# Adamtaranto/mimeo

Hardware: AMD Instinct MI355X
Metric: Gbp-aligned/sec (mimeo self, 1 Gbp genome, --minIdt 80 --minLen 100 --minCov 3) (higher is better)
Workload: dtype int32

## Files before the change

mimeo_amd/csrc/k6.h:

```cpp
#pragma once
#include <algorithm>
#include <cstdio>
#include <cstdlib>
#include <vector>

#include "device_util.h"

namespace mimeo {

constexpr int32_t NEG = -(1 << 30);
constexpr int32_t NEGH = -(1 << 29);

struct Cell {
    int32_t s;
    uint32_t nm, nx;
};
struct HalfResult {
    int32_t score;
    uint32_t i, j, nm, nx, overflow;
    uint32_t maxcols, rows;
    uint32_t base_lo, base_hi;
};
struct DpJob {
    uint32_t group, at, aq;
// ... 108 lines not shown
            const uint32_t side = t >= (long long)an.x ? 1u : 0u;
            const uint2 ix = B.P.pidx[2u * (b0 + rank) + side];
            const bool traced = ix.x != PATH_UNTRACED;
            const uint32_t n = traced ? ix.y : 0u;
            const PathBlock *blk = B.P.blk + (traced ? ix.x : 0u);
            const uint32_t lo = blocks_upto(blk, n, t);
            PathBlock b{0, 0, 0};
            if (lo) b = blk[lo - 1];
            if (lo && t - (long long)b.t < (long long)b.len) {
                const long long d = (long long)b.q - (long long)b.t, k = dir > 0 ? d - d0 : d0 - d;
                if (k <= 0) kmin = max(kmin, k);
                if (k >= 0) kmax = min(kmax, k);
                c = dir > 0 ? (long long)b.t + b.len : (long long)b.t - 1;
            } else if (dir > 0) {
                c = lo < n ? (long long)blk[lo].t : (side == 0 ? (long long)an.x : (long long)o.tend);
            } else {
                c = lo ? (long long)b.t + b.len - 1 : (side == 1 ? (long long)an.x - 1 : (long long)o.tstart - 1);
            }
        } else if (dir > 0) {
            c = (long long)o.tstart > t ? (long long)o.tstart : K_INF;
        } else {
            c = (long long)o.tend <= t ? (long long)o.tend - 1 : -1;
        }
        nt = dir > 0 ? min(nt, c) : max(nt, c);
    }
    for (int o = 32; o > 0; o >>= 1) {
        kmin = max(kmin, __shfl_xor(kmin, o));
        kmax = min(kmax, __shfl_xor(kmax, o));
        const long long on = __shfl_xor(nt, o);
        nt = dir > 0 ? min(nt, on) : max(nt, on);
    }
    RowBound r;
    r.kmin = wave_uniform_ll(kmin); r.kmax = wave_uniform_ll(kmax);
    nt = wave_uniform_ll(nt);
    const long long nrow = dir > 0 ? nt - (long long)at + 1 : (long long)at - nt;
    r.next = nrow > 0xFFFFFFFEll ? 0xFFFFFFFFu : (uint32_t)nrow;
    r.any = (r.kmin > -K_INF || r.kmax < K_INF) ? 1u : 0u;
    return r;
}
__device__ __forceinline__ bool bounds_none(const BoundCtx &B, uint64_t b0, uint32_t nacc, uint32_t at, int dir) {
    bool hit = false;
    for (uint32_t e = threadIdx.x & 63u; e < nacc; e += 64u) {
        const mimeo_alignment o = B.aln[b0 + e];
        if (o.tend > o.tstart && (dir > 0 ? o.tend > at : o.tstart < at)) hit = true;
    }
    return __ballot(hit) == 0;
}

struct K6Buffers {
    DeviceBuf anchors, packed, jobs, res, cnt, astate, ovf_list, any;
    DeviceBuf pidx, accrank, arena, pool, tjobs, tres, tctr;
    DeviceBuf kjobs, pcnt, pslot, ptmp;
    DeviceBuf sweep;
};
extern K6Buffers g_k6;
int dp_round(Group *d_groups, uint32_t n, const mimeo_params *p, int32_t cap, bool bounded, const BoundCtx &bc, unsigned int *novf, unsigned int *nrestart);
int arena_reserve(uint64_t blocks, uint64_t used);
struct TraceStats { uint64_t arena_used, largest; float ms; uint32_t slices; };
int trace_round(Group *d_groups, const DpJob *d_jobs, uint32_t h0, const mimeo_params *p, int32_t cap, uint64_t budget, TraceStats &ts, bool bounded, BoundCtx bc);
int paths_pass(Group *d_groups, uint32_t ngroups, const mimeo_params *p, int32_t cap, const mimeo_alignment *d_aln, uint64_t budget, bool k6_stats);

}
```

mimeo_amd/csrc/k6_dp.hip:

```cpp
#include "k6_band.h"

namespace mimeo {

template <int WSTRIP>
__device__ __forceinline__ void load_qbits(const GStrandView &Q, uint32_t aq, int dir, uint32_t jb, uint32_t lenB,
                                           uint32_t &qlo, uint32_t &qhi, uint32_t &qn) {
    constexpr uint32_t SMASK = WSTRIP == 32 ? 0xFFFFFFFFu : ((1u << (WSTRIP & 31)) - 1u);
    if (jb > lenB) { qlo = qhi = qn = 0; return; }
    if (dir > 0) {
        int32_t p = (int32_t)(aq + jb) - 1;
        const Win32 w = win32(Q, p);
        qlo = w.lo & SMASK; qhi = w.hi & SMASK; qn = w.nm & SMASK;
    } else {
        int32_t p = (int32_t)aq - (int32_t)jb - (WSTRIP - 1);
        const Win32 w = win32(Q, p);
        qlo = __brev(w.lo & SMASK) >> (32 - WSTRIP); qhi = __brev(w.hi & SMASK) >> (32 - WSTRIP);
        qn = __brev(w.nm & SMASK) >> (32 - WSTRIP);
    }
}

struct RowBases { uint32_t lo, hi, nm; };
__device__ __forceinline__ RowBases load_row_bases(const GStrandView &T, uint32_t at, int dir, uint32_t i0) {
    if (dir > 0) {
        const Win32 w = win32(T, (int32_t)(at + i0 - 1u));
// ... 505 lines not shown
    return AnyRow{(int32_t *)b, (int32_t *)(b + ANY_COLS), b + 2u * ANY_COLS, b + 3u * ANY_COLS, b + 4u * ANY_COLS, b + 5u * ANY_COLS};
}
constexpr size_t ANY_SLOT_WORDS = 2u * 6u * (size_t)ANY_COLS;

struct CountRows {
    static constexpr uint32_t M = ANY_COLS - 1u, W = ANY_COLS;
    uint32_t *base;
    AnyRow P, N;
    __device__ __forceinline__ BandRows rows(uint32_t par, uint32_t, uint32_t) {
        P = any_row(base, par); N = any_row(base, par ^ 1u);
        return BandRows{P.cs, P.ds, N.cs, N.ds};
    }
    __device__ __forceinline__ void init(uint32_t j, int32_t c) {
        const AnyRow r0 = any_row(base, 0);
        r0.cs[j & M] = c; r0.cm[j & M] = 0; r0.cx[j & M] = 0;
        r0.ds[j & M] = NEG; r0.dm[j & M] = 0; r0.dx[j & M] = 0;
    }
    __device__ __forceinline__ Cell h(uint32_t j, bool dlive, bool dopen, bool diag, bool m, bool hd) const {
        Cell dd{0, 0, 0}, g{0, 0, 0};
        if (dlive) { dd.nm = P.dm[j & M]; dd.nx = P.dx[j & M]; }
        if (dopen) { dd.nm = P.cm[j & M]; dd.nx = P.cx[j & M]; }
        if (diag) { g.nm = P.cm[(j - 1) & M] + (m ? 1u : 0u); g.nx = P.cx[(j - 1) & M] + (m ? 0u : 1u); }
        N.dm[j & M] = dd.nm; N.dx[j & M] = dd.nx;
        const Cell hh = hd ? dd : g;
        N.cm[j & M] = hh.nm; N.cx[j & M] = hh.nx;
        return hh;
    }
    __device__ __forceinline__ Cell htag(uint32_t j) const { return Cell{0, N.cm[j & M], N.cx[j & M]}; }
    __device__ __forceinline__ Cell c(uint32_t j, const Cell &ht, const Cell &ia, bool ci) const { const Cell ct = ci ? ia : ht; N.cm[j & M] = ct.nm; N.cx[j & M] = ct.nx; return ct; }
};

template <bool BOUND>
__global__ __launch_bounds__(ANY_THREADS) void k6_dp_any(const Group *__restrict__ groups, const DpJob *__restrict__ jobs,
                                                         const unsigned int *__restrict__ list, uint32_t first,
                                                         HalfResult *__restrict__ res, uint32_t *__restrict__ scratch,
                                                         int32_t O, int32_t E, int32_t Y, int32_t cap, BoundCtx B,
                                                         HalfSweep *__restrict__ sweep) {
    const DpJob job = jobs[list[first + blockIdx.x]];
    const Group &G = groups[job.group];
    const uint32_t lenA = job.dir > 0 ? G.T.len - job.at : job.at;
    CountRows rows{scratch + (size_t)blockIdx.x * ANY_SLOT_WORDS};
    HalfSweep sw;
    const HalfResult r = band_dp<ANY_THREADS, BOUND>(rows, G, job, lenA, O, E, Y, cap, B, sw);
    if (threadIdx.x == 0) res[job.slot] = r;
    if (BOUND && threadIdx.x == 0) sweep[job.slot] = sw;
}

__global__ void k6_list_all(uint32_t n, unsigned int *__restrict__ novf, unsigned int *__restrict__ ovf_list) {
    const uint32_t k = blockIdx.x * blockDim.x + threadIdx.x;
    if (k < n) ovf_list[k] = k;
    if (k == 0) *novf = n;
}

int dp_round(Group *d_groups, uint32_t n, const mimeo_params *p, int32_t cap, bool bounded, const BoundCtx &bc,
                    unsigned int *novf, unsigned int *nrestart) {
    hipStream_t st = stream();
    int rc;
    const Group *groups = d_groups;
    const DpJob *jobs = (const DpJob *)g_k6.jobs.p;
    HalfResult *res = (HalfResult *)g_k6.res.p;
    HalfSweep *sweep = bounded ? (HalfSweep *)g_k6.sweep.p : nullptr;
    unsigned int *list = (unsigned int *)g_k6.ovf_list.p;
    const int32_t O = p->gap_open, E = p->gap_extend, Y = p->ydrop;
    const bool lean_ok = E <= (1 << 16) && O <= (1 << 24) && Y <= (1 << 28);
    if (bounded) {
        if (lean_ok) hipLaunchKernelGGL(k6_dp1_bounded, dim3(n), dim3(64), 0, st, groups, jobs, res, sweep, O, E, Y, bc, novf, list);
        else hipLaunchKernelGGL(k6_list_all, dim3((n + 255) / 256), dim3(256), 0, st, n, novf, list);
    } else {
        if (lean_ok) hipLaunchKernelGGL(k6_dp1, dim3(n), dim3(64), 0, st, groups, jobs, res, O, E, Y, nrestart);
        hipLaunchKernelGGL(k6_dp_wide, dim3(n), dim3(64), 0, st, groups, jobs, res, O, E, Y, novf, list, cap, lean_ok ? 0 : 1);
    }
    unsigned int nov = 0;
    HIP_TRY(hipMemcpyAsync(&nov, novf, 4, hipMemcpyDeviceToHost, st));
    HIP_TRY(hipStreamSynchronize(st));
    if (!nov) return 0;
    const unsigned int slots = std::min<unsigned int>(nov, 32u);
    if ((rc = g_k6.any.reserve((size_t)slots * ANY_SLOT_WORDS * 4))) return rc;
    const auto any = bounded ? k6_dp_any<true> : k6_dp_any<false>;
    for (unsigned int f = 0; f < nov; f += slots)
        hipLaunchKernelGGL(any, dim3(std::min(slots, nov - f)), dim3(ANY_THREADS), 0, st, groups, jobs, (const unsigned int *)list, f, res,
                           (uint32_t *)g_k6.any.p, O, E, Y, cap, bc, sweep);
    return 0;
}

}
```

mimeo_amd/csrc/k6_gapped.hip:

```cpp
#include "k6.h"

namespace mimeo {

constexpr uint32_t ANCHOR_W = 31, ANCHOR_CHUNK = 4096;
constexpr int ANCHOR_THREADS = 1024;

__device__ void wave_anchor_chunk(const GStrandView &T, const GStrandView &Q, const mimeo_hsp &h, uint32_t chunk,
                                  unsigned long long *packed) {
    const uint32_t lane = threadIdx.x & 63u, nw = h.length - ANCHOR_W + 1;
    const int32_t d = (int32_t)h.tstart - (int32_t)h.qstart;
    const uint32_t w0 = chunk * ANCHOR_CHUNK + lane * (ANCHOR_CHUNK / 64u), w1 = min(nw, w0 + ANCHOR_CHUNK / 64u);
    int32_t bs = INT32_MIN;
    uint32_t bw = 0xFFFFFFFFu;
    if (w0 < w1) {
        int32_t sum = 0;
        bool m;
        for (uint32_t k = 0; k < ANCHOR_W; k++) {
            int32_t pt = (int32_t)(h.tstart + w0 + k);
            sum += pair_score(T, Q, pt, pt - d, &m);
        }
        bs = sum; bw = w0;
        for (uint32_t w = w0 + 1; w < w1; w++) {
            int32_t add = (int32_t)(h.tstart + w + ANCHOR_W - 1), sub = (int32_t)(h.tstart + w - 1);
            sum += pair_score(T, Q, add, add - d, &m) - pair_score(T, Q, sub, sub - d, &m);
            if (sum > bs) { bs = sum; bw = w; }
        }
    }
    for (int o = 32; o > 0; o >>= 1) {
        int32_t ob = __shfl_xor(bs, o);
        uint32_t ow = __shfl_xor(bw, o);
        if (ob > bs || (ob == bs && ow < bw)) { bs = ob; bw = ow; }
    }
    if (lane == 0 && bw != 0xFFFFFFFFu)
        atomicMax(packed, ((unsigned long long)(uint32_t)(bs + 8192) << 32) | (unsigned long long)(0xFFFFFFFFu - bw));
}

constexpr uint32_t ANCHOR_SPLIT = 16;
__global__ __launch_bounds__(ANCHOR_THREADS) void k6_anchor_points(const Group *__restrict__ groups,
                                                                   const mimeo_hsp *__restrict__ hs,
                                                                   const uint32_t *__restrict__ order,
                                                                   unsigned long long *__restrict__ packed) {
    const Group &G = groups[blockIdx.x];
    const uint64_t b0 = G.hsp_begin;
    const uint32_t nw = gridDim.y * (ANCHOR_THREADS / 64), me = blockIdx.y * (ANCHOR_THREADS / 64) + (threadIdx.x >> 6);
    uint32_t item = 0;
    for (uint32_t r = 0; r < G.nchain; r++) {
        const mimeo_hsp h = hs[b0 + order[b0 + r]];
        if (h.length <= ANCHOR_W) continue;
        const uint32_t nch = (h.length - ANCHOR_W + 1 + ANCHOR_CHUNK - 1) / ANCHOR_CHUNK;
        const uint32_t first = (me + nw - item % nw) % nw;
        for (uint32_t c = first; c < nch; c += nw) wave_anchor_chunk(G.T, G.Q, h, c, &packed[b0 + r]);
        item += nch;
    }
}
__global__ __launch_bounds__(256) void k6_anchor_final(const Group *__restrict__ groups, const mimeo_hsp *__restrict__ hs,
                                                       const uint32_t *__restrict__ order,
                                                       const unsigned long long *__restrict__ packed,
                                                       uint2 *__restrict__ anchors) {
    const Group &G = groups[blockIdx.x];
    const uint64_t b0 = G.hsp_begin;
    for (uint32_t r = threadIdx.x; r < G.nchain; r += blockDim.x) {
        const mimeo_hsp h = hs[b0 + order[b0 + r]];
        uint32_t off = h.length / 2;
        if (h.length > ANCHOR_W) off = (0xFFFFFFFFu - (uint32_t)packed[b0 + r]) + ANCHOR_W / 2;
        anchors[b0 + r] = make_uint2(h.tstart + off, h.qstart + off);
    }
}

__device__ __forceinline__ bool in_boxes(const mimeo_alignment *aln, uint32_t n, uint2 a) {
    bool inside = false;
    for (uint32_t e = threadIdx.x & 63u; e < n; e += 64u) {
        const mimeo_alignment &o = aln[e];
        if (a.x >= o.tstart && a.x < o.tend && a.y >= o.qstart && a.y < o.qend) inside = true;
    }
    return __ballot(inside) != 0;
}

__device__ __forceinline__ bool on_half_path(const PathBlock *blk, uint32_t n, uint2 a) {
    const uint32_t lo = blocks_upto(blk, n, a.x);
    if (!lo) return false;
    const PathBlock b = blk[lo - 1];
    return a.x - b.t < b.len && a.y >= b.q && a.y - b.q == a.x - b.t;
}
__device__ __forceinline__ bool on_path(const PathView &P, const uint2 *anchors, uint64_t b0, uint32_t rank, uint2 a) {
    const uint2 an = anchors[b0 + rank];
    const uint2 ix = P.pidx[2u * (b0 + rank) + (a.x >= an.x ? 1u : 0u)];
    if (ix.x == PATH_UNTRACED) return false;
    return on_half_path(P.blk + ix.x, ix.y, a);
}
template <bool PATH>
__device__ __forceinline__ bool skip_test(const mimeo_alignment *aln, uint32_t n, uint2 a, const PathView &P,
                                          const uint2 *anchors, uint64_t b0) {
    if (!PATH) return in_boxes(aln + b0, n, a);
    bool on = false;
    for (uint32_t e = threadIdx.x & 63u; e < n; e += 64u) {
        const mimeo_alignment &o = aln[b0 + e];
        if (a.x >= o.tstart && a.x < o.tend && a.y >= o.qstart && a.y < o.qend && on_path(P, anchors, b0, P.accrank[b0 + e], a))
            on = true;
    }
    return __ballot(on) != 0;
}

enum : uint8_t { A_NEW = 0, A_DONE = 1, A_SKIPPED = 2, A_ACCEPTED = 3 };
constexpr uint32_t PICK_SCAN = 2048;
constexpr uint32_t NEAR_DIAG = 256, NEAR_POS = 8192, MAX_DEFER = 2;
constexpr uint32_t GUARD_FREE = 32, GUARD_DIAG = 4096, GUARD_COUNT = 4;

__device__ __forceinline__ uint32_t anchor_relation(uint2 a, uint2 b) {
    int32_t da = (int32_t)a.x - (int32_t)a.y, db = (int32_t)b.x - (int32_t)b.y;
    uint32_t dd = (uint32_t)abs(da - db), dp = a.x > b.x ? a.x - b.x : b.x - a.x;
    return ((dd <= NEAR_DIAG && dp <= NEAR_POS) ? 1u : 0u) | (dd <= GUARD_DIAG ? 2u : 0u);
}

template <bool PATH>
__global__ __launch_bounds__(64) void k6_pick(Group *__restrict__ groups, const uint2 *__restrict__ anchors,
                                              const mimeo_alignment *__restrict__ aln, uint32_t bmax,
                                              uint8_t *__restrict__ astate, uint8_t *__restrict__ adefer,
                                              DpJob *__restrict__ jobs, unsigned int *__restrict__ njobs, PathView P) {
    __shared__ uint32_t sb[MAX_BATCH];
    Group &G = groups[blockIdx.x];
    const uint64_t b0 = G.hsp_begin;
    const uint32_t first = G.next, lane = threadIdx.x;
    uint32_t nb = 0;
    for (uint32_t r = first; r < G.nchain && nb < bmax && r - first < PICK_SCAN; r++) {
        if (astate[b0 + r] != A_NEW) continue;
        const uint2 a = anchors[b0 + r];
        if (skip_test<PATH>(aln, G.nacc, a, P, anchors, b0)) {
            if (lane == 0) astate[b0 + r] = A_SKIPPED;
            continue;
        }
        uint32_t near = 0, band = 0;
        for (uint32_t r2 = first + lane; r2 < r; r2 += 64)
            if (astate[b0 + r2] == A_DONE) { const uint32_t x = anchor_relation(a, anchors[b0 + r2]); near |= x & 1u; band += x >> 1; }
        for (uint32_t k = lane; k < nb; k += 64) { const uint32_t x = anchor_relation(a, anchors[b0 + sb[k]]); near |= x & 1u; band += x >> 1; }
        if (__ballot(near) && adefer[b0 + r] < MAX_DEFER) {
            if (lane == 0) adefer[b0 + r]++;
            continue;
        }
        if (nb >= GUARD_FREE) {
            for (int o = 32; o > 0; o >>= 1) band += __shfl_xor(band, o);
            if (band >= GUARD_COUNT) continue;
        }
        if (lane == 0) sb[nb] = r;
        nb++;
        __syncthreads();
    }
    if (lane == 0) {
        G.nbatch = nb;
        unsigned int j0 = nb ? atomicAdd(njobs, 2u * nb) : 0u;
        G.job0 = j0;
        for (uint32_t k = 0; k < nb; k++) {
            const uint32_t r = sb[k];
            astate[b0 + r] = A_DONE;
            const uint2 a = anchors[b0 + r];
            const uint32_t slot = 2u * (uint32_t)(b0 + r);
            jobs[j0 + 2 * k] = DpJob{blockIdx.x, a.x, a.y, -1, slot, 0};
            jobs[j0 + 2 * k + 1] = DpJob{blockIdx.x, a.x, a.y, +1, slot + 1, 0};
        }
    }
}

constexpr uint32_t RESOLVE_NEW = 256;
static_assert(RESOLVE_NEW >= (uint32_t)MAX_BATCH, "k6_resolve accepts a full take in one invocation");

__device__ __forceinline__ bool bounds_touch(const PathView &P, const uint2 *anchors, uint64_t b0, uint32_t rank, uint4 o, uint2 a,
                                             const HalfResult &L, const HalfResult &R, const HalfSweep &sL, const HalfSweep &sR) {
    const uint32_t rowsL = L.rows ? L.rows : L.i, rowsR = R.rows ? R.rows : R.i;
    const long long tlo = (long long)a.x - rowsL, thi = (long long)a.x + rowsR;
    if ((long long)o.y <= tlo || (long long)o.x >= thi) return false;
    const long long d0 = (long long)a.y - (long long)a.x;
    bool hit = false;
    for (uint32_t side = 0; side < 2; side++) {
        const uint2 ix = P.pidx[2u * (b0 + rank) + side];
        if (ix.x == PATH_UNTRACED) continue;
        for (uint32_t k = threadIdx.x & 63u; k < ix.y; k += 64u) {
            const PathBlock b = P.blk[ix.x + k];
            const long long t0 = b.t, t1 = (long long)b.t + b.len, d = (long long)b.q - (long long)b.t;
            if (t0 < thi && t1 > (long long)a.x && d - d0 >= sR.klo && d - d0 <= sR.khi) hit = true;
            if (t0 < (long long)a.x && t1 > tlo && d0 - d >= sL.klo && d0 - d <= sL.khi) hit = true;
        }
    }
    return __ballot(hit) != 0;
}

template <bool PATH, bool BOUND = false, bool RANK = false>
__global__ __launch_bounds__(64) void k6_resolve(Group *__restrict__ groups, const uint2 *__restrict__ anchors,
                                                 const HalfResult *__restrict__ res, mimeo_alignment *__restrict__ aln,
                                                 uint8_t *__restrict__ astate, unsigned int *__restrict__ remaining, PathView P,
                                                 const HalfSweep *__restrict__ sweep) {
    __shared__ uint4 sbox[RESOLVE_NEW];
    __shared__ uint32_t srank[PATH ? RESOLVE_NEW : 1];
    Group &G = groups[blockIdx.x];
    const uint64_t b0 = G.hsp_begin;
    const uint32_t nacc0 = G.nacc;
    uint32_t nnew = 0, overflow = 0, r = G.next;
    for (; r < G.nchain; r++) {
        const uint8_t st = astate[b0 + r];
        if (st == A_SKIPPED || st == A_ACCEPTED) continue;
        if (nnew == RESOLVE_NEW) break;
        const uint2 a = anchors[b0 + r];
        bool inside = skip_test<PATH>(aln, nacc0, a, P, anchors, b0);
        if (!inside) {
            bool in2 = false;
            for (uint32_t e = threadIdx.x; e < nnew; e += 64) {
                uint4 o = sbox[e];
                if (a.x >= o.x && a.x < o.y && a.y >= o.z && a.y < o.w && (!PATH || on_path(P, anchors, b0, srank[PATH ? e : 0], a)))
                    in2 = true;
            }
            inside = __ballot(in2) != 0;
        }
// ... 103 lines not shown
            const uint32_t v = threadIdx.x >= o ? part[threadIdx.x - o] : 0u;
            __syncthreads();
            part[threadIdx.x] += v;
            __syncthreads();
        }
        if (g < ngroups) groups[g].job0 = carry + part[threadIdx.x] - n;
        __syncthreads();
        if (threadIdx.x == 1023) carry += part[1023];
        __syncthreads();
    }
}
__global__ __launch_bounds__(64) void k6_dense_copy(const Group *__restrict__ groups, const mimeo_alignment *__restrict__ aln,
                                                    mimeo_alignment *__restrict__ dense) {
    const Group &G = groups[blockIdx.x];
    for (uint32_t k = threadIdx.x; k < G.naln; k += 64) dense[G.job0 + k] = aln[G.hsp_begin + k];
}
void dense_alignments_device(Group *d_groups, uint32_t ngroups, const mimeo_alignment *d_aln, mimeo_alignment *d_dense) {
    hipLaunchKernelGGL(k6_dense_offsets, dim3(1), dim3(1024), 0, stream(), d_groups, ngroups);
    hipLaunchKernelGGL(k6_dense_copy, dim3(ngroups), dim3(64), 0, stream(), (const Group *)d_groups, d_aln, d_dense);
}

__global__ void k6_kept_ranks(Group *__restrict__ groups, uint32_t ngroups, const mimeo_alignment *__restrict__ aln,
                              uint32_t *__restrict__ accrank, const uint2 *__restrict__ pidx, int32_t thresh) {
    const uint32_t g = blockIdx.x * blockDim.x + threadIdx.x;
    if (g >= ngroups) return;
    Group &G = groups[g];
    const uint64_t b0 = G.hsp_begin;
    uint32_t k = 0;
    for (uint32_t e = 0; e < G.nacc; e++) {
        if (aln[b0 + e].score < thresh) continue;
        const uint32_t rank = accrank[b0 + e];
        const uint32_t slot = 2u * (uint32_t)(b0 + rank);
        if (pidx[slot].x == PATH_UNTRACED || pidx[slot + 1].x == PATH_UNTRACED) G.overflow = 1;
        accrank[b0 + k++] = rank;
    }
}

__global__ __launch_bounds__(256) void k6_ungapped_paths(const Group *__restrict__ groups, const mimeo_alignment *__restrict__ aln,
                                                         PathBlock *__restrict__ arena, uint2 *__restrict__ pidx,
                                                         uint32_t *__restrict__ accrank) {
    const Group &G = groups[blockIdx.x];
    const uint64_t b0 = G.hsp_begin;
    for (uint32_t r = threadIdx.x; r < G.nacc; r += 256) {
        const mimeo_alignment a = aln[b0 + r];
        arena[b0 + r] = PathBlock{a.tstart, a.qstart, a.tend - a.tstart};
        pidx[2u * (b0 + r)] = make_uint2((uint32_t)(b0 + r), 1u);
        pidx[2u * (b0 + r) + 1u] = make_uint2(0u, 0u);
        accrank[b0 + r] = r;
    }
}

K6Buffers g_k6;

static int round_stats(uint32_t n, uint64_t nhsps, bool bounded, unsigned long long *bound_jobs, const unsigned int *nrestart) {
    std::vector<DpJob> hj(n);
    std::vector<HalfResult> hall((size_t)nhsps * 2), hr(n);
    HIP_TRY(hipStreamSynchronize(stream()));
    HIP_TRY(hipMemcpy(hj.data(), g_k6.jobs.p, (size_t)n * sizeof(DpJob), hipMemcpyDeviceToHost));
    HIP_TRY(hipMemcpy(hall.data(), g_k6.res.p, hall.size() * sizeof(HalfResult), hipMemcpyDeviceToHost));
    for (size_t k = 0; k < hr.size(); k++) hr[k] = hall[hj[k].slot];
    unsigned long long hist[9] = {0}, rows = 0, maxr = 0, shortcut = 0;
    for (auto &r : hr) {
        if (!r.rows) { shortcut++; continue; }
        hist[std::min<uint32_t>(8, r.maxcols / 128)]++; rows += r.rows; maxr = std::max<unsigned long long>(maxr, r.rows);
    }
    unsigned long long rebased = 0;
    for (auto &r : hr) if (r.base_lo | r.base_hi) rebased++;
    unsigned int wide[2] = {0, 0};
    HIP_TRY(hipMemcpy(wide, nrestart, 8, hipMemcpyDeviceToHost));
    fprintf(stderr, "[k6] full strip width: restarted %u widened %u of %u\n", wide[0], wide[1], n);
    fprintf(stderr, "[k6] jobs %u shortcut %llu (rebased in k6_dp_any: %llu) rows total %llu max %llu band<128..>=1024:", n, shortcut, rebased, rows, maxr);
    for (int b = 0; b < 9; b++) fprintf(stderr, " %llu", hist[b]);
    fprintf(stderr, "\n");
    {
        unsigned long long fine[34] = {0};
        for (auto &r : hr) if (r.rows) fine[std::min<uint32_t>(33, r.maxcols / 32)]++;
        fprintf(stderr, "[k6] widest band, buckets of 32 columns from 448:");
        for (int b = 14; b < 34; b++) fprintf(stderr, " %llu", fine[b]);
        fprintf(stderr, "\n");
    }
    if (n <= 8)
        for (size_t k = 0; k < hr.size(); k++)
            fprintf(stderr, "  [k6] job %zu: dir %d rows %u maxcols %u i %u j %u rebased %d\n", k, hj[k].dir, hr[k].rows, hr[k].maxcols, hr[k].i, hr[k].j,
                    (hr[k].base_lo | hr[k].base_hi) ? 1 : 0);
    int shown = 0;
    for (auto &r : hr)
        if (!r.rows && shown < 8) { fprintf(stderr, "  [k6] zero-row job: score %d i %u j %u nm %u nx %u ovf %u\n", r.score, r.i, r.j, r.nm, r.nx, r.overflow); shown++; }
    if (bounded) {
        std::vector<HalfSweep> hs((size_t)nhsps * 2);
        HIP_TRY(hipMemcpy(hs.data(), g_k6.sweep.p, hs.size() * sizeof(HalfSweep), hipMemcpyDeviceToHost));
        for (auto &j : hj) *bound_jobs += hs[j.slot].nbound ? 1u : 0u;
    }
    return 0;
}

static int accepted_stats(const Group *d_groups, uint32_t ngroups, uint32_t bmax) {
    std::vector<Group> hg(ngroups);
    HIP_TRY(hipStreamSynchronize(stream()));
    HIP_TRY(hipMemcpy(hg.data(), d_groups, (size_t)ngroups * sizeof(Group), hipMemcpyDeviceToHost));
    unsigned long long hist[11] = {0}, sum = 0, over = 0;
    uint32_t mx = 0;
    for (const Group &g : hg) {
        uint32_t b = 0;
        while (b < 10 && (b ? 1u << (b - 1) : 0u) < g.nacc) b++;
        hist[b]++; sum += g.nacc; mx = std::max(mx, g.nacc); over += g.nacc > bmax ? 1u : 0u;
    }
    fprintf(stderr, "[k6] accepted per group: max %u mean %.2f of %u groups, %llu above the take of %u; 0 1 2 <=4 <=8 .. <=256 more:", mx,
            (double)sum / ngroups, ngroups, over, bmax);
    for (int b = 0; b < 11; b++) fprintf(stderr, " %llu", hist[b]);
    fprintf(stderr, "\n");
    return 0;
}

struct K6Call {
    uint32_t bmax, rounds;
    bool stats, path, bounded, box_paths;
    int32_t cap;
    uint64_t pool_budget;
    unsigned long long bound_jobs, rescheduled;
    TraceStats ts;
};

static int gapped_setup(Group *d_groups, uint32_t ngroups, const mimeo_hsp *d_sorted, const uint32_t *d_order, uint64_t nhsps, K6Call &c) {
    c.bmax = getenv("MIMEO_K6_BMAX") ? (uint32_t)atoi(getenv("MIMEO_K6_BMAX")) : K6_ROUND_ANCHORS / ngroups;
    c.bmax = c.bmax < 1 ? 1 : (c.bmax > MAX_BATCH ? MAX_BATCH : c.bmax);
    c.stats = getenv("MIMEO_K6_STATS") != nullptr;
    if (c.stats) fprintf(stderr, "[k6] take %u anchors per group and round (%u groups, limit %d, budget %u)\n", c.bmax, ngroups, MAX_BATCH, K6_ROUND_ANCHORS);
    c.cap = getenv("MIMEO_K6_SCORE_CAP") ? std::max(100000, atoi(getenv("MIMEO_K6_SCORE_CAP"))) : 2000000000;
    hipStream_t st = stream();
    int rc;
    if ((rc = g_k6.anchors.reserve(nhsps * sizeof(uint2)))) return rc;
    if ((rc = g_k6.packed.reserve(nhsps * 8))) return rc;
    HIP_TRY(hipMemsetAsync(g_k6.packed.p, 0, nhsps * 8, st));
    if ((rc = g_k6.jobs.reserve((size_t)ngroups * c.bmax * 2 * sizeof(DpJob)))) return rc;
    if ((rc = g_k6.res.reserve((size_t)nhsps * 2 * sizeof(HalfResult)))) return rc;
    if ((rc = g_k6.astate.reserve((size_t)nhsps * 2))) return rc;
    HIP_TRY(hipMemsetAsync(g_k6.astate.p, 0, (size_t)nhsps * 2, st));
    if ((rc = g_k6.cnt.reserve(32))) return rc;
    if ((rc = g_k6.ovf_list.reserve((size_t)ngroups * c.bmax * 2 * sizeof(unsigned int)))) return rc;
    const uint32_t asplit = ngroups > 4096 ? 1u : ANCHOR_SPLIT;
    hipLaunchKernelGGL(k6_anchor_points, dim3(ngroups, asplit), dim3(ANCHOR_THREADS), 0, st, (const Group *)d_groups,
                       d_sorted, d_order, (unsigned long long *)g_k6.packed.p);
    hipLaunchKernelGGL(k6_anchor_final, dim3(ngroups), dim3(256), 0, st, (const Group *)d_groups, d_sorted, d_order,
                       (const unsigned long long *)g_k6.packed.p, (uint2 *)g_k6.anchors.p);
    if (c.path || c.box_paths) {
        if ((rc = g_k6.tctr.reserve(16))) return rc;
        if ((rc = arena_reserve(1024, 0))) return rc;
        HIP_TRY(hipMemsetAsync(g_k6.tctr.p, 0, 16, st));
        size_t free_b = 0, total_b = 0;
        HIP_TRY(hipMemGetInfo(&free_b, &total_b));
        c.pool_budget = std::min<uint64_t>(((uint64_t)free_b + g_k6.pool.cap) / 4, 16ull << 30);
        if (getenv("MIMEO_K6_TRACE_POOL_MB")) c.pool_budget = (uint64_t)atol(getenv("MIMEO_K6_TRACE_POOL_MB")) << 20;
    }
    if (c.bounded && (rc = g_k6.sweep.reserve((size_t)nhsps * 2 * sizeof(HalfSweep)))) return rc;
    return 0;
}

static int gapped_rounds(Group *d_groups, uint32_t ngroups, uint64_t nhsps, const mimeo_params *p, mimeo_alignment *d_aln, K6Call &c) {
    hipStream_t st = stream();
    int rc;
    PathView pv{nullptr, nullptr, nullptr};
    if (c.path || c.box_paths) pv = PathView{(const uint2 *)g_k6.pidx.p, nullptr, (uint32_t *)g_k6.accrank.p};
    const auto pick = c.path ? k6_pick<true> : k6_pick<false>;
    const auto resolve = c.bounded ? k6_resolve<true, true> : c.path ? k6_resolve<true, false>
                         : c.box_paths ? k6_resolve<false, false, true> : k6_resolve<false, false>;
    const HalfSweep *sweep = c.bounded ? (const HalfSweep *)g_k6.sweep.p : nullptr;
    for (;;) {
        HIP_TRY(hipMemsetAsync(g_k6.cnt.p, 0, 32, st));
        unsigned int *njobs = (unsigned int *)g_k6.cnt.p, *remaining = njobs + 1, *novf = njobs + 2, *nrestart = njobs + 4;
        pv.blk = (const PathBlock *)g_k6.arena.p;
        hipLaunchKernelGGL(pick, dim3(ngroups), dim3(64), 0, st, d_groups, (const uint2 *)g_k6.anchors.p, (const mimeo_alignment *)d_aln,
                           c.bmax, (uint8_t *)g_k6.astate.p, (uint8_t *)g_k6.astate.p + nhsps, (DpJob *)g_k6.jobs.p, njobs, pv);
        unsigned int h0 = 0;
        HIP_TRY(hipMemcpyAsync(&h0, njobs, 4, hipMemcpyDeviceToHost, st));
        HIP_TRY(hipStreamSynchronize(st));
        if (h0) {
            const BoundCtx bc{(const mimeo_alignment *)d_aln, (const uint2 *)g_k6.anchors.p, pv};
            if ((rc = dp_round(d_groups, h0, p, c.cap, c.bounded, bc, novf, nrestart))) return rc;
            if (c.stats && (rc = round_stats(h0, nhsps, c.bounded, &c.bound_jobs, nrestart))) return rc;
            if (c.path) {
                c.rounds++;
                if ((rc = trace_round(d_groups, (const DpJob *)g_k6.jobs.p, h0, p, c.cap, c.pool_budget, c.ts, c.bounded, bc))) return rc;
                pv.blk = (const PathBlock *)g_k6.arena.p;
            }
        }
        hipLaunchKernelGGL(resolve, dim3(ngroups), dim3(64), 0, st, d_groups, (const uint2 *)g_k6.anchors.p, (const HalfResult *)g_k6.res.p,
                           d_aln, (uint8_t *)g_k6.astate.p, remaining, pv, sweep);
        unsigned int h4[4] = {0, 0, 0, 0};
        HIP_TRY(hipMemcpyAsync(h4, g_k6.cnt.p, 16, hipMemcpyDeviceToHost, st));
        HIP_TRY(hipStreamSynchronize(st));
        c.rescheduled += h4[3];
        if (!h4[1]) return 0;
    }
}

static void path_rule_stats(const K6Call &c) {
    fprintf(stderr, "[k6] path rule: traceback %.3f ms, rounds %u slices %u, %llu path blocks, pool %.1f MB, largest half %.3f MB", c.ts.ms,
            c.rounds, c.ts.slices, (unsigned long long)c.ts.arena_used, g_k6.pool.cap / 1048576.0, c.ts.largest / 1048576.0);
    if (c.bounded) fprintf(stderr, ", bounded jobs %llu, rescheduled %llu", c.bound_jobs, c.rescheduled);
    fprintf(stderr, "\n");
}

int gapped_device(Group *d_groups, uint32_t ngroups, const mimeo_hsp *d_sorted, const uint32_t *d_order,
                  uint64_t nhsps, const mimeo_params *p, mimeo_alignment *d_aln, bool want_paths) {
    if (!ngroups || !nhsps) return 0;
    hipStream_t st = stream();
    int rc;
    const bool path = p->gapped && p->anchor_rule == MIMEO_ANCHOR_PATH;
    if (want_paths && nhsps >= (1ull << 31)) { set_error("paths: more than 2^31 HSPs in one batch"); return MIMEO_ERR_LIMIT; }
    if (want_paths || path) {
        if ((rc = g_k6.pidx.reserve((size_t)nhsps * 2 * sizeof(uint2)))) return rc;
        if ((rc = g_k6.accrank.reserve((size_t)nhsps * 4))) return rc;
    }
    if (!p->gapped) {
        hipLaunchKernelGGL(k6_ungapped, dim3(ngroups), dim3(256), 0, st, d_groups, d_sorted, d_order, d_aln);
        if (want_paths) {
            if ((rc = arena_reserve(nhsps, 0))) return rc;
            hipLaunchKernelGGL(k6_ungapped_paths, dim3(ngroups), dim3(256), 0, st, (const Group *)d_groups, (const mimeo_alignment *)d_aln,
                               (PathBlock *)g_k6.arena.p, (uint2 *)g_k6.pidx.p, (uint32_t *)g_k6.accrank.p);
        }
    } else {
        K6Call c{};
        c.path = path; c.box_paths = want_paths && !path; c.bounded = path && p->bound_extensions;
        if ((rc = gapped_setup(d_groups, ngroups, d_sorted, d_order, nhsps, c))) return rc;
        if ((rc = gapped_rounds(d_groups, ngroups, nhsps, p, d_aln, c))) return rc;
        if (c.stats && (rc = accepted_stats(d_groups, ngroups, c.bmax))) return rc;
        if (c.path && c.stats) path_rule_stats(c);
        if (c.box_paths && (rc = paths_pass(d_groups, ngroups, p, c.cap, d_aln, c.pool_budget, c.stats))) return rc;
    }
    if (want_paths)
        hipLaunchKernelGGL(k6_kept_ranks, dim3((ngroups + 63) / 64), dim3(64), 0, st, d_groups, ngroups, (const mimeo_alignment *)d_aln,
                           (uint32_t *)g_k6.accrank.p, (const uint2 *)g_k6.pidx.p, p->hspthresh);
    hipLaunchKernelGGL(k6_finish, dim3((ngroups + 63) / 64), dim3(64), 0, st, d_groups, ngroups, d_aln, p->hspthresh);
    HIP_TRY(hipGetLastError());
    return 0;
// ... 4 lines not shown
```

Before: 0.05260.

## Parallelize anchor window scan with wave prefix sums and add optional DP job ordering

The anchor search now assigns one column per lane and uses a wave-wide inclusive prefix sum to score all 31-base windows at once, where before each lane slid its own window over a contiguous slice. Chunk distribution across waves is reworked with a shared-memory prefix over HSP chunk counts and a binary search, replacing the per-HSP serial loop. It also records per-anchor reach and a padding estimate in each DP job, and adds an env-selected job ordering (longest or shortest first) using a simple O(n^2) rank sort. The default order is unchanged, so the main intended change to timing is the restructured anchor kernel, with some extra shared-memory traffic and barriers.

```diff
diff --git a/mimeo_amd/csrc/anchor_window.h b/mimeo_amd/csrc/anchor_window.h
--- /dev/null
+++ b/mimeo_amd/csrc/anchor_window.h
@@ -0,0 +1,85 @@
+#pragma once
+#include <cstdint>
+
+#if defined(__HIPCC__) || defined(__CUDACC__)
+#define ANCHOR_WINDOW_FN __host__ __device__ inline __attribute__((always_inline))
+#else
+#define ANCHOR_WINDOW_FN inline
+#endif
+
+namespace mimeo {
+namespace anchor_window {
+
+constexpr uint32_t W = 31, BLOCK = 64, CHUNK = 4096;
+constexpr int32_t BIAS = 8192;
+constexpr uint32_t NO_START = 0xFFFFFFFFu;
+constexpr int32_t NO_SUM = INT32_MIN;
+static_assert(W < BLOCK && CHUNK % BLOCK == 0, "G(c - W) lies in this block or in the one before");
+
+ANCHOR_WINDOW_FN uint32_t windows(uint32_t length) { return length > W ? length - W + 1 : 0u; }
+ANCHOR_WINDOW_FN uint32_t chunks(uint32_t length) { return (windows(length) + CHUNK - 1) / CHUNK; }
+ANCHOR_WINDOW_FN uint32_t first_start(uint32_t chunk) { return chunk * CHUNK; }
+ANCHOR_WINDOW_FN uint32_t end_start(uint32_t length, uint32_t chunk) {
+    const uint32_t nw = windows(length), e = first_start(chunk) + CHUNK;
+    return e < nw ? e : nw;
+}
+ANCHOR_WINDOW_FN uint32_t blocks(uint32_t length, uint32_t chunk) {
+    const uint32_t w0 = first_start(chunk), w1 = end_start(length, chunk);
+    return w1 > w0 ? (w1 - w0 + W - 1 + BLOCK - 1) / BLOCK : 0u;
+}
+ANCHOR_WINDOW_FN uint32_t column(uint32_t chunk, uint32_t block, uint32_t lane) { return first_start(chunk) + block * BLOCK + lane; }
+ANCHOR_WINDOW_FN bool ends_a_window(uint32_t length, uint32_t chunk, uint32_t col) {
+    return col >= first_start(chunk) + W - 1 && col - (W - 1) < end_start(length, chunk);
+}
+ANCHOR_WINDOW_FN uint32_t start_of_window_ending(uint32_t col) { return col - (W - 1); }
+ANCHOR_WINDOW_FN uint32_t below_lane(uint32_t lane) { return (lane + BLOCK - W) & (BLOCK - 1); }
+ANCHOR_WINDOW_FN bool below_in_previous(uint32_t lane) { return lane < W; }
+
+ANCHOR_WINDOW_FN bool better(int32_t bsum, uint32_t bstart, int32_t asum, uint32_t astart) {
+    return bsum > asum || (bsum == asum && bstart < astart);
+}
+ANCHOR_WINDOW_FN unsigned long long pack(int32_t sum, uint32_t start) {
+    return ((unsigned long long)(uint32_t)(sum + BIAS) << 32) | (unsigned long long)(0xFFFFFFFFu - start);
+}
+ANCHOR_WINDOW_FN uint32_t anchor_offset(uint32_t length, unsigned long long packed) {
+    return length > W ? (0xFFFFFFFFu - (uint32_t)packed) + W / 2 : length / 2;
+}
+
+template <class Score>
+inline unsigned long long chunk_packed(Score score, uint32_t length, uint32_t chunk) {
+    int32_t g[BLOCK], prev[BLOCK], bs[BLOCK];
+    uint32_t bw[BLOCK];
+    for (uint32_t l = 0; l < BLOCK; l++) { prev[l] = 0; bs[l] = NO_SUM; bw[l] = NO_START; }
+    int32_t carry = 0;
+    const uint32_t nb = blocks(length, chunk);
+    for (uint32_t b = 0; b < nb; b++) {
+        for (uint32_t l = 0; l < BLOCK; l++) {
+            const uint32_t col = column(chunk, b, l);
+            carry += col < length ? score(col) : 0;
+            g[l] = carry;
+        }
+        for (uint32_t l = 0; l < BLOCK; l++) {
+            const uint32_t col = column(chunk, b, l), src = below_lane(l);
+            const int32_t sum = g[l] - (below_in_previous(l) ? prev[src] : g[src]);
+            if (ends_a_window(length, chunk, col) && sum > bs[l]) { bs[l] = sum; bw[l] = start_of_window_ending(col); }
+        }
+        for (uint32_t l = 0; l < BLOCK; l++) prev[l] = g[l];
+    }
+    int32_t s = NO_SUM;
+    uint32_t w = NO_START;
+    for (uint32_t l = 0; l < BLOCK; l++)
+        if (better(bs[l], bw[l], s, w)) { s = bs[l]; w = bw[l]; }
+    return w == NO_START ? 0ull : pack(s, w);
+}
+template <class Score>
+inline uint32_t anchor_offset_of(Score score, uint32_t length) {
+    unsigned long long best = 0;
+    for (uint32_t c = chunks(length); c-- > 0;) {
+        const unsigned long long p = chunk_packed(score, length, c);
+        if (p > best) best = p;
+    }
+    return anchor_offset(length, best);
+}
+
+}
+}
diff --git a/mimeo_amd/csrc/k6.h b/mimeo_amd/csrc/k6.h
--- a/mimeo_amd/csrc/k6.h
+++ b/mimeo_amd/csrc/k6.h
@@ -184,9 +184,10 @@
     DeviceBuf pidx, accrank, arena, pool, tjobs, tres, tctr;
     DeviceBuf kjobs, pcnt, pslot, ptmp;
     DeviceBuf sweep;
+    DeviceBuf reach, keys, jobs2;
 };
 extern K6Buffers g_k6;
-int dp_round(Group *d_groups, uint32_t n, const mimeo_params *p, int32_t cap, bool bounded, const BoundCtx &bc, unsigned int *novf, unsigned int *nrestart);
+int dp_round(Group *d_groups, const DpJob *jobs, uint32_t n, const mimeo_params *p, int32_t cap, bool bounded, const BoundCtx &bc, unsigned int *novf, unsigned int *nrestart);
 int arena_reserve(uint64_t blocks, uint64_t used);
 struct TraceStats { uint64_t arena_used, largest; float ms; uint32_t slices; };
 int trace_round(Group *d_groups, const DpJob *d_jobs, uint32_t h0, const mimeo_params *p, int32_t cap, uint64_t budget, TraceStats &ts, bool bounded, BoundCtx bc);
diff --git a/mimeo_amd/csrc/k6_dp.hip b/mimeo_amd/csrc/k6_dp.hip
--- a/mimeo_amd/csrc/k6_dp.hip
+++ b/mimeo_amd/csrc/k6_dp.hip
@@ -581,12 +581,11 @@
     if (k == 0) *novf = n;
 }
 
-int dp_round(Group *d_groups, uint32_t n, const mimeo_params *p, int32_t cap, bool bounded, const BoundCtx &bc,
-                    unsigned int *novf, unsigned int *nrestart) {
+int dp_round(Group *d_groups, const DpJob *jobs, uint32_t n, const mimeo_params *p, int32_t cap, bool bounded, const BoundCtx &bc,
+             unsigned int *novf, unsigned int *nrestart) {
     hipStream_t st = stream();
     int rc;
     const Group *groups = d_groups;
-    const DpJob *jobs = (const DpJob *)g_k6.jobs.p;
     HalfResult *res = (HalfResult *)g_k6.res.p;
     HalfSweep *sweep = bounded ? (HalfSweep *)g_k6.sweep.p : nullptr;
     unsigned int *list = (unsigned int *)g_k6.ovf_list.p;
diff --git a/mimeo_amd/csrc/k6_gapped.hip b/mimeo_amd/csrc/k6_gapped.hip
--- a/mimeo_amd/csrc/k6_gapped.hip
+++ b/mimeo_amd/csrc/k6_gapped.hip
@@ -1,38 +1,37 @@
+#include <cstring>
+
+#include "anchor_window.h"
 #include "k6.h"
 
 namespace mimeo {
 
-constexpr uint32_t ANCHOR_W = 31, ANCHOR_CHUNK = 4096;
+namespace aw = anchor_window;
 constexpr int ANCHOR_THREADS = 1024;
 
-__device__ void wave_anchor_chunk(const GStrandView &T, const GStrandView &Q, const mimeo_hsp &h, uint32_t chunk,
-                                  unsigned long long *packed) {
-    const uint32_t lane = threadIdx.x & 63u, nw = h.length - ANCHOR_W + 1;
-    const int32_t d = (int32_t)h.tstart - (int32_t)h.qstart;
-    const uint32_t w0 = chunk * ANCHOR_CHUNK + lane * (ANCHOR_CHUNK / 64u), w1 = min(nw, w0 + ANCHOR_CHUNK / 64u);
-    int32_t bs = INT32_MIN;
-    uint32_t bw = 0xFFFFFFFFu;
-    if (w0 < w1) {
-        int32_t sum = 0;
+__device__ void wave_anchor_chunk(const GStrandView &T, const GStrandView &Q, uint32_t tstart, uint32_t qstart, uint32_t length,
+                                  uint32_t chunk, unsigned long long *packed) {
+    const uint32_t lane = threadIdx.x & 63u, nb = aw::blocks(length, chunk), src = aw::below_lane(lane);
+    const bool from_prev = aw::below_in_previous(lane);
+    int32_t bs = aw::NO_SUM, prev = 0, carry = 0;
+    uint32_t bw = aw::NO_START;
+    for (uint32_t b = 0; b < nb; b++) {
+        const uint32_t col = aw::column(chunk, b, lane);
+        int32_t s = 0;
         bool m;
-        for (uint32_t k = 0; k < ANCHOR_W; k++) {
-            int32_t pt = (int32_t)(h.tstart + w0 + k);
-            sum += pair_score(T, Q, pt, pt - d, &m);
-        }
-        bs = sum; bw = w0;
-        for (uint32_t w = w0 + 1; w < w1; w++) {
-            int32_t add = (int32_t)(h.tstart + w + ANCHOR_W - 1), sub = (int32_t)(h.tstart + w - 1);
-            sum += pair_score(T, Q, add, add - d, &m) - pair_score(T, Q, sub, sub - d, &m);
-            if (sum > bs) { bs = sum; bw = w; }
-        }
+        if (col < length) s = pair_score(T, Q, (int32_t)(tstart + col), (int32_t)(qstart + col), &m);
+        const int32_t g = carry + (int32_t)wave_inclusive_sum((uint32_t)s);
+        const int32_t gc = __shfl(g, (int)src), gp = __shfl(prev, (int)src);
+        const int32_t sum = g - (from_prev ? gp : gc);
+        if (aw::ends_a_window(length, chunk, col) && sum > bs) { bs = sum; bw = aw::start_of_window_ending(col); }
+        carry = __builtin_amdgcn_readlane(g, 63);
+        prev = g;
     }
     for (int o = 32; o > 0; o >>= 1) {
         int32_t ob = __shfl_xor(bs, o);
         uint32_t ow = __shfl_xor(bw, o);
-        if (ob > bs || (ob == bs && ow < bw)) { bs = ob; bw = ow; }
-    }
-    if (lane == 0 && bw != 0xFFFFFFFFu)
-        atomicMax(packed, ((unsigned long long)(uint32_t)(bs + 8192) << 32) | (unsigned long long)(0xFFFFFFFFu - bw));
+        if (aw::better(ob, ow, bs, bw)) { bs = ob; bw = ow; }
+    }
+    if (lane == 0 && bw != aw::NO_START) atomicMax(packed, aw::pack(bs, bw));
 }
 
 constexpr uint32_t ANCHOR_SPLIT = 16;
@@ -40,30 +39,51 @@
                                                                    const mimeo_hsp *__restrict__ hs,
                                                                    const uint32_t *__restrict__ order,
                                                                    unsigned long long *__restrict__ packed) {
+    __shared__ uint32_t s_t[ANCHOR_THREADS], s_q[ANCHOR_THREADS], s_len[ANCHOR_THREADS], s_pre[ANCHOR_THREADS];
+    __shared__ uint32_t s_wave[ANCHOR_THREADS / 64];
     const Group &G = groups[blockIdx.x];
     const uint64_t b0 = G.hsp_begin;
-    const uint32_t nw = gridDim.y * (ANCHOR_THREADS / 64), me = blockIdx.y * (ANCHOR_THREADS / 64) + (threadIdx.x >> 6);
+    const uint32_t nw = gridDim.y * (ANCHOR_THREADS / 64), wave = threadIdx.x >> 6, me = blockIdx.y * (ANCHOR_THREADS / 64) + wave;
     uint32_t item = 0;
-    for (uint32_t r = 0; r < G.nchain; r++) {
-        const mimeo_hsp h = hs[b0 + order[b0 + r]];
-        if (h.length <= ANCHOR_W) continue;
-        const uint32_t nch = (h.length - ANCHOR_W + 1 + ANCHOR_CHUNK - 1) / ANCHOR_CHUNK;
-        const uint32_t first = (me + nw - item % nw) % nw;
-        for (uint32_t c = first; c < nch; c += nw) wave_anchor_chunk(G.T, G.Q, h, c, &packed[b0 + r]);
-        item += nch;
+    for (uint32_t r0 = 0; r0 < G.nchain; r0 += ANCHOR_THREADS) {
+        const uint32_t r = r0 + threadIdx.x;
+        uint32_t nch = 0;
+        if (r < G.nchain) {
+            const mimeo_hsp h = hs[b0 + order[b0 + r]];
+            s_t[threadIdx.x] = h.tstart; s_q[threadIdx.x] = h.qstart; s_len[threadIdx.x] = h.length;
+            nch = aw::chunks(h.length);
+        }
+        const uint32_t inc = wave_inclusive_sum(nch);
+        if ((threadIdx.x & 63u) == 63u) s_wave[wave] = inc;
+        __syncthreads();
+        uint32_t before = 0, total = 0;
+        for (uint32_t w = 0; w < ANCHOR_THREADS / 64; w++) { const uint32_t c = s_wave[w]; before += w < wave ? c : 0u; total += c; }
+        s_pre[threadIdx.x] = before + inc;
+        __syncthreads();
+        for (uint32_t i = (me + nw - item) % nw; i < total; i += nw) {
+            uint32_t lo = 0, hi = ANCHOR_THREADS - 1;
+            while (lo < hi) {
+                const uint32_t mid = (lo + hi) >> 1;
+                if (s_pre[mid] > i) hi = mid; else lo = mid + 1;
+            }
+            const uint32_t chunk = i - (lo ? s_pre[lo - 1] : 0u);
+            wave_anchor_chunk(G.T, G.Q, s_t[lo], s_q[lo], s_len[lo], chunk, &packed[b0 + r0 + lo]);
+        }
+        item = (item + total % nw) % nw;
+        __syncthreads();
     }
 }
 __global__ __launch_bounds__(256) void k6_anchor_final(const Group *__restrict__ groups, const mimeo_hsp *__restrict__ hs,
                                                        const uint32_t *__restrict__ order,
                                                        const unsigned long long *__restrict__ packed,
-                                                       uint2 *__restrict__ anchors) {
+                                                       uint2 *__restrict__ anchors, uint2 *__restrict__ reach) {
     const Group &G = groups[blockIdx.x];
     const uint64_t b0 = G.hsp_begin;
     for (uint32_t r = threadIdx.x; r < G.nchain; r += blockDim.x) {
         const mimeo_hsp h = hs[b0 + order[b0 + r]];
-        uint32_t off = h.length / 2;
-        if (h.length > ANCHOR_W) off = (0xFFFFFFFFu - (uint32_t)packed[b0 + r]) + ANCHOR_W / 2;
+        const uint32_t off = aw::anchor_offset(h.length, packed[b0 + r]);
         anchors[b0 + r] = make_uint2(h.tstart + off, h.qstart + off);
+        reach[b0 + r] = make_uint2(off, h.length - off);
     }
 }
 
@@ -112,12 +132,16 @@
     return ((dd <= NEAR_DIAG && dp <= NEAR_POS) ? 1u : 0u) | (dd <= GUARD_DIAG ? 2u : 0u);
 }
 
+constexpr uint32_t PAD_CAP = 0xFFFFu;
+
 template <bool PATH>
 __global__ __launch_bounds__(64) void k6_pick(Group *__restrict__ groups, const uint2 *__restrict__ anchors,
+                                              const uint2 *__restrict__ reach,
                                               const mimeo_alignment *__restrict__ aln, uint32_t bmax,
                                               uint8_t *__restrict__ astate, uint8_t *__restrict__ adefer,
                                               DpJob *__restrict__ jobs, unsigned int *__restrict__ njobs, PathView P) {
     __shared__ uint32_t sb[MAX_BATCH];
+    __shared__ uint32_t sfar[2][MAX_BATCH];
     Group &G = groups[blockIdx.x];
     const uint64_t b0 = G.hsp_begin;
     const uint32_t first = G.next, lane = threadIdx.x;
@@ -132,7 +156,12 @@
         uint32_t near = 0, band = 0;
         for (uint32_t r2 = first + lane; r2 < r; r2 += 64)
             if (astate[b0 + r2] == A_DONE) { const uint32_t x = anchor_relation(a, anchors[b0 + r2]); near |= x & 1u; band += x >> 1; }
-        for (uint32_t k = lane; k < nb; k += 64) { const uint32_t x = anchor_relation(a, anchors[b0 + sb[k]]); near |= x & 1u; band += x >> 1; }
+        for (uint32_t k = lane; k < nb; k += 64) {
+            const uint2 s = anchors[b0 + sb[k]];
+            const uint32_t x = anchor_relation(a, s);
+            near |= x & 1u; band += x >> 1;
+            if (x & 1u) { const uint32_t side = a.x >= s.x ? 1u : 0u; sfar[side][k] = max(sfar[side][k], side ? a.x - s.x : s.x - a.x); }
+        }
         if (__ballot(near) && adefer[b0 + r] < MAX_DEFER) {
             if (lane == 0) adefer[b0 + r]++;
             continue;
@@ -141,10 +170,11 @@
             for (int o = 32; o > 0; o >>= 1) band += __shfl_xor(band, o);
             if (band >= GUARD_COUNT) continue;
         }
-        if (lane == 0) sb[nb] = r;
+        if (lane == 0) { sb[nb] = r; sfar[0][nb] = 0; sfar[1][nb] = 0; }
         nb++;
         __syncthreads();
     }
+    __syncthreads();
     if (lane == 0) {
         G.nbatch = nb;
         unsigned int j0 = nb ? atomicAdd(njobs, 2u * nb) : 0u;
@@ -154,8 +184,9 @@
             astate[b0 + r] = A_DONE;
             const uint2 a = anchors[b0 + r];
             const uint32_t slot = 2u * (uint32_t)(b0 + r);
-            jobs[j0 + 2 * k] = DpJob{blockIdx.x, a.x, a.y, -1, slot, 0};
-            jobs[j0 + 2 * k + 1] = DpJob{blockIdx.x, a.x, a.y, +1, slot + 1, 0};
+            const uint2 own = reach[b0 + r];
+            jobs[j0 + 2 * k] = DpJob{blockIdx.x, a.x, a.y, -1, slot, min(PAD_CAP, max(own.x, sfar[0][k]))};
+            jobs[j0 + 2 * k + 1] = DpJob{blockIdx.x, a.x, a.y, +1, slot + 1, min(PAD_CAP, max(own.y, sfar[1][k]))};
         }
     }
 }
@@ -365,11 +396,42 @@
 
 K6Buffers g_k6;
 
-static int round_stats(uint32_t n, uint64_t nhsps, bool bounded, unsigned long long *bound_jobs, const unsigned int *nrestart) {
+enum : int { ORDER_PICK = 0, ORDER_LONGEST = 1, ORDER_SHORTEST = 2 };
+static const char *const ORDER_NAME[3] = {"pick", "longest", "shortest"};
+__global__ __launch_bounds__(256) void k6_order_keys(const DpJob *__restrict__ jobs, uint32_t n, int order,
+                                                     unsigned long long *__restrict__ keys) {
+    const uint32_t k = blockIdx.x * blockDim.x + threadIdx.x;
+    if (k >= n) return;
+    const uint32_t pad = min(jobs[k].pad, PAD_CAP);
+    keys[k] = ((unsigned long long)(order == ORDER_LONGEST ? PAD_CAP - pad : pad) << 32) | jobs[k].slot;
+}
+__global__ __launch_bounds__(256) void k6_order_place(const DpJob *__restrict__ jobs, const unsigned long long *__restrict__ keys,
+                                                      uint32_t n, DpJob *__restrict__ sorted) {
+    const uint32_t k = blockIdx.x * blockDim.x + threadIdx.x;
+    const unsigned long long mine = k < n ? keys[k] : 0ull;
+    uint32_t rank = 0;
+    for (uint32_t j = 0; j < n; j++) rank += keys[j] < mine ? 1u : 0u;
+    if (k < n) sorted[rank] = jobs[k];
+}
+static int order_jobs(uint32_t n, int order, const DpJob **round_jobs) {
+    *round_jobs = (const DpJob *)g_k6.jobs.p;
+    if (order == ORDER_PICK) return 0;
+    int rc;
+    if ((rc = g_k6.keys.reserve((size_t)n * 8))) return rc;
+    if ((rc = g_k6.jobs2.reserve((size_t)n * sizeof(DpJob)))) return rc;
+    hipLaunchKernelGGL(k6_order_keys, dim3((n + 255) / 256), dim3(256), 0, stream(), (const DpJob *)g_k6.jobs.p, n, order,
+                       (unsigned long long *)g_k6.keys.p);
+    hipLaunchKernelGGL(k6_order_place, dim3((n + 255) / 256), dim3(256), 0, stream(), (const DpJob *)g_k6.jobs.p,
+                       (const unsigned long long *)g_k6.keys.p, n, (DpJob *)g_k6.jobs2.p);
+    *round_jobs = (const DpJob *)g_k6.jobs2.p;
+    return 0;
+}
+
+static int round_stats(const DpJob *d_jobs, int order, uint32_t n, uint64_t nhsps, bool bounded, unsigned long long *bound_jobs, const unsigned int *nrestart) {
     std::vector<DpJob> hj(n);
     std::vector<HalfResult> hall((size_t)nhsps * 2), hr(n);
     HIP_TRY(hipStreamSynchronize(stream()));
-    HIP_TRY(hipMemcpy(hj.data(), g_k6.jobs.p, (size_t)n * sizeof(DpJob), hipMemcpyDeviceToHost));
+    HIP_TRY(hipMemcpy(hj.data(), d_jobs, (size_t)n * sizeof(DpJob), hipMemcpyDeviceToHost));
     HIP_TRY(hipMemcpy(hall.data(), g_k6.res.p, hall.size() * sizeof(HalfResult), hipMemcpyDeviceToHost));
     for (size_t k = 0; k < hr.size(); k++) hr[k] = hall[hj[k].slot];
     unsigned long long hist[9] = {0}, rows = 0, maxr = 0, shortcut = 0;
@@ -404,6 +466,9 @@
         HIP_TRY(hipMemcpy(hs.data(), g_k6.sweep.p, hs.size() * sizeof(HalfSweep), hipMemcpyDeviceToHost));
         for (auto &j : hj) *bound_jobs += hs[j.slot].nbound ? 1u : 0u;
     }
+    fprintf(stderr, "[k6-order] %s: pad of the %u jobs in launch order:", ORDER_NAME[order], n);
+    for (auto &j : hj) fprintf(stderr, " %u", j.pad);
+    fprintf(stderr, "\n");
     return 0;
 }
 
@@ -427,6 +492,7 @@
 
 struct K6Call {
     uint32_t bmax, rounds;
+    int order;
     bool stats, path, bounded, box_paths;
     int32_t cap;
     uint64_t pool_budget;
@@ -438,11 +504,18 @@
     c.bmax = getenv("MIMEO_K6_BMAX") ? (uint32_t)atoi(getenv("MIMEO_K6_BMAX")) : K6_ROUND_ANCHORS / ngroups;
     c.bmax = c.bmax < 1 ? 1 : (c.bmax > MAX_BATCH ? MAX_BATCH : c.bmax);
     c.stats = getenv("MIMEO_K6_STATS") != nullptr;
+    c.order = ORDER_PICK;
+    if (const char *o = getenv("MIMEO_K6_ORDER")) {
+        c.order = -1;
+        for (int k = 0; k < 3; k++) if (!strcmp(o, ORDER_NAME[k])) c.order = k;
+        if (c.order < 0) { set_error("MIMEO_K6_ORDER must be pick, longest or shortest"); return MIMEO_ERR_ARG; }
+    }
+    int rc;
     if (c.stats) fprintf(stderr, "[k6] take %u anchors per group and round (%u groups, limit %d, budget %u)\n", c.bmax, ngroups, MAX_BATCH, K6_ROUND_ANCHORS);
     c.cap = getenv("MIMEO_K6_SCORE_CAP") ? std::max(100000, atoi(getenv("MIMEO_K6_SCORE_CAP"))) : 2000000000;
     hipStream_t st = stream();
-    int rc;
     if ((rc = g_k6.anchors.reserve(nhsps * sizeof(uint2)))) return rc;
+    if ((rc = g_k6.reach.reserve(nhsps * sizeof(uint2)))) return rc;
     if ((rc = g_k6.packed.reserve(nhsps * 8))) return rc;
     HIP_TRY(hipMemsetAsync(g_k6.packed.p, 0, nhsps * 8, st));
     if ((rc = g_k6.jobs.reserve((size_t)ngroups * c.bmax * 2 * sizeof(DpJob)))) return rc;
@@ -455,7 +528,7 @@
     hipLaunchKernelGGL(k6_anchor_points, dim3(ngroups, asplit), dim3(ANCHOR_THREADS), 0, st, (const Group *)d_groups,
                        d_sorted, d_order, (unsigned long long *)g_k6.packed.p);
     hipLaunchKernelGGL(k6_anchor_final, dim3(ngroups), dim3(256), 0, st, (const Group *)d_groups, d_sorted, d_order,
-                       (const unsigned long long *)g_k6.packed.p, (uint2 *)g_k6.anchors.p);
+                       (const unsigned long long *)g_k6.packed.p, (uint2 *)g_k6.anchors.p, (uint2 *)g_k6.reach.p);
     if (c.path || c.box_paths) {
         if ((rc = g_k6.tctr.reserve(16))) return rc;
         if ((rc = arena_reserve(1024, 0))) return rc;
@@ -482,18 +555,20 @@
         HIP_TRY(hipMemsetAsync(g_k6.cnt.p, 0, 32, st));
         unsigned int *njobs = (unsigned int *)g_k6.cnt.p, *remaining = njobs + 1, *novf = njobs + 2, *nrestart = njobs + 4;
         pv.blk = (const PathBlock *)g_k6.arena.p;
-        hipLaunchKernelGGL(pick, dim3(ngroups), dim3(64), 0, st, d_groups, (const uint2 *)g_k6.anchors.p, (const mimeo_alignment *)d_aln,
+        hipLaunchKernelGGL(pick, dim3(ngroups), dim3(64), 0, st, d_groups, (const uint2 *)g_k6.anchors.p, (const uint2 *)g_k6.reach.p, (const mimeo_alignment *)d_aln,
                            c.bmax, (uint8_t *)g_k6.astate.p, (uint8_t *)g_k6.astate.p + nhsps, (DpJob *)g_k6.jobs.p, njobs, pv);
         unsigned int h0 = 0;
         HIP_TRY(hipMemcpyAsync(&h0, njobs, 4, hipMemcpyDeviceToHost, st));
         HIP_TRY(hipStreamSynchronize(st));
         if (h0) {
             const BoundCtx bc{(const mimeo_alignment *)d_aln, (const uint2 *)g_k6.anchors.p, pv};
-            if ((rc = dp_round(d_groups, h0, p, c.cap, c.bounded, bc, novf, nrestart))) return rc;
-            if (c.stats && (rc = round_stats(h0, nhsps, c.bounded, &c.bound_jobs, nrestart))) return rc;
+            const DpJob *round_jobs;
+            if ((rc = order_jobs(h0, c.order, &round_jobs))) return rc;
+            if ((rc = dp_round(d_groups, round_jobs, h0, p, c.cap, c.bounded, bc, novf, nrestart))) return rc;
+            if (c.stats && (rc = round_stats(round_jobs, c.order, h0, nhsps, c.bounded, &c.bound_jobs, nrestart))) return rc;
             if (c.path) {
                 c.rounds++;
-                if ((rc = trace_round(d_groups, (const DpJob *)g_k6.jobs.p, h0, p, c.cap, c.pool_budget, c.ts, c.bounded, bc))) return rc;
+                if ((rc = trace_round(d_groups, round_jobs, h0, p, c.cap, c.pool_budget, c.ts, c.bounded, bc))) return rc;
                 pv.blk = (const PathBlock *)g_k6.arena.p;
             }
         }
```

Result: no change. 0.05298 (median of 6 runs) (+0.7%).
